# SrikarK-code/clip-dplm

Hardware: NVIDIA B200
Metric: contrastive_fwd_bwd_pairs_per_sec (higher is better)
Workload: dtype bf16

## Files before the change

### clip-dplm_b200/csrc/clipnce_api.cu

```cuda
#include <cuda.h>
#include <cuda_bf16.h>
#include <cuda_runtime.h>

#include <cmath>
#include <cstdarg>
#include <cstdio>
#include <cstdlib>
#include <cstring>
#include <mutex>
#include <set>
#include <string>
#include <utility>

#include "../../include/clipnce.h"
#include "kernels_aux.cuh"
#include "kernels_head.cuh"
#include "kernels_link.cuh"
#include "kernels_pair.cuh"
#include "kernels_pair2.cuh"
#include "kernels_simt.cuh"
#include "kernels_tc.cuh"

namespace {

thread_local std::string g_err;

int fail(int code, const char* fmt, ...) {
  char buf[512];
  va_list ap;
  va_start(ap, fmt);
  vsnprintf(buf, sizeof buf, fmt, ap);
  va_end(ap);
  g_err = buf;
  return code;
}

#define CUDA_TRY(expr)                                                                              \
  do {                                                                                              \
    cudaError_t e_ = (expr);                                                                        \
    if (e_ != cudaSuccess) return fail(CLIPNCE_ECUDA, "%s: %s", #expr, cudaGetErrorString(e_));     \
  } while (0)

long long env_int(const char* name, long long dflt) {
  const char* e = getenv(name);
  return e ? atoll(e) : dflt;
}

unsigned long long link_timeout_ns() {
  static const unsigned long long ns = [] {
    const long long ms = env_int("CLIPNCE_LINK_TIMEOUT_MS", 600000);
    return (unsigned long long)(ms > 0 ? ms : 600000) * 1000000ull;
  }();
  return ns;
}
inline cudaStream_t as_stream(void* s) { return reinterpret_cast<cudaStream_t>(s); }
inline int64_t ceil_div(int64_t a, int64_t b) { return (a + b - 1) / b; }
inline int64_t round_up(int64_t a, int64_t b) { return ceil_div(a, b) * b; }
inline bool aligned16(const void* p) { return (reinterpret_cast<uintptr_t>(p) & 15u) == 0; }
inline size_t elem_size(int dtype) { return dtype == CLIPNCE_BF16 ? 2 : 4; }

bool pair_eligible(int64_t d) { return d % 128 == 0 && d >= 128 && d <= 768; }

int tc_family(int dtype, int64_t d, float scale, int flags) {
  if (dtype != CLIPNCE_BF16 || (flags & CLIPNCE_FLAG_FORCE_EXACT) || d < 8 || d % 8 != 0 || d > 768 || !(scale > 0.f)) return 0;
  if (!(flags & CLIPNCE_FLAG_UNBOUNDED) && 2.f * scale <= 80.f) return 1;
  return pair_eligible(d) ? 2 : 0;
}
bool tc_eligible(int dtype, int64_t d, float scale, int flags) { return tc_family(dtype, d, scale, flags) == 1; }

typedef CUresult (*EncodeTiledFn)(CUtensorMap*, CUtensorMapDataType, cuuint32_t, void*, const cuuint64_t*,
                                  const cuuint64_t*, const cuuint32_t*, const cuuint32_t*, CUtensorMapInterleave,
                                  CUtensorMapSwizzle, CUtensorMapL2promotion, CUtensorMapFloatOOBfill);
std::mutex g_mu;
EncodeTiledFn g_encode = nullptr;
std::set<std::pair<const void*, int>> g_smem_allowed;

int get_encode(EncodeTiledFn* out) {
  std::lock_guard<std::mutex> lk(g_mu);
  if (!g_encode) {
    void* fn = nullptr;
    cudaDriverEntryPointQueryResult qres;
    CUDA_TRY(cudaGetDriverEntryPoint("cuTensorMapEncodeTiled", &fn, cudaEnableDefault, &qres));
    if (qres != cudaDriverEntryPointSuccess || fn == nullptr)
      return fail(CLIPNCE_ECUDA, "cuTensorMapEncodeTiled not available from this driver");
    g_encode = reinterpret_cast<EncodeTiledFn>(fn);
  }
  *out = g_encode;
  return 0;
}

int make_tmap(CUtensorMap* m, const void* base, int64_t inner, int64_t outer, int64_t ld, int box_rows) {
  EncodeTiledFn enc;
  int rc = get_encode(&enc);
  if (rc) return rc;
  cuuint64_t dims[2] = {(cuuint64_t)inner, (cuuint64_t)outer};
  cuuint64_t strides[1] = {(cuuint64_t)ld * 2};
  cuuint32_t box[2] = {64u, (cuuint32_t)box_rows};
  cuuint32_t estr[2] = {1u, 1u};
  CUresult r = enc(m, CU_TENSOR_MAP_DATA_TYPE_BFLOAT16, 2, const_cast<void*>(base), dims, strides, box, estr,
                   CU_TENSOR_MAP_INTERLEAVE_NONE, CU_TENSOR_MAP_SWIZZLE_128B, CU_TENSOR_MAP_L2_PROMOTION_L2_256B,
                   CU_TENSOR_MAP_FLOAT_OOB_FILL_NONE);
  if (r != CUDA_SUCCESS)
// ... 950 lines not shown
    }
    if (world >= 2 || forced_seg >= 1) break;
  }
  if (best_p == 0) return false;
  pl->P = best_p;
  pl->Q = slots - best_p;
  pl->n_seg = best_seg;
  pl->seg_steps = pl->n_steps / best_seg;
  pl->n_items = pl->n_rb * best_seg;
  pl->n_rounds = (int)ceil_div(pl->n_items, pl->P);
  pl->depth = pair2::RING_DEPTH;
  const int nkc = (int)(d / 64);
  const int total = (pair::SMEM_LIMIT - pair2::producer_smem(nkc, 0)) / pair::STAGE_BYTES;
  if (total < 4) return false;
  auto cap = [](int v) { return v > pair2::MAXS ? pair2::MAXS : v; };
  pl->stages_b = cap(total / 2);
  pl->stages_a = cap(total - total / 2);
  pl->stages_c = cap((pair::SMEM_LIMIT - pair2::consumer_smem(0)) / pair2::C_STAGE);
  const int ps = pair2::producer_smem(nkc, pl->stages_a + pl->stages_b), cs = pair2::consumer_smem(pl->stages_c);
  pl->smem = ps > cs ? ps : cs;
  size_t off = 0;
  auto region = [&](size_t bytes) { const size_t o = off; off = (size_t)round_up((int64_t)(off + bytes), 256); return o; };
  pl->off_flags = region(sizeof(uint32_t) * 2 * (size_t)pl->n_rounds * (size_t)pl->seg_steps);
  pl->off_ring = region((size_t)pl->depth * (size_t)pl->P * 128 * 256 * 2);
  pl->off_dxh = region(sizeof(float) * (size_t)pl->n_seg * (size_t)n_rows * (size_t)d);
  pl->off_dyh = region(sizeof(float) * (size_t)n_cols * (size_t)d);
  pl->off_part = region(sizeof(float) * (size_t)ceil_div(n_rows > n_cols ? n_rows : n_cols, 8));
  pl->bytes = off;
  return true;
}

int launch_finish(const float* parts, int n_split, int64_t slab_elems, const void* xc, const void* xo, int in_dtype,
                  const float* rinv, const float* grad_scale, int64_t n, int64_t d, void* dx, int out_dtype, float* ds_part,
                  cudaStream_t st) {
  const unsigned grid = (unsigned)ceil_div(n, 8);
  const size_t smem = sizeof(float) * 8 * (size_t)d;
  const int di = (int)d;
#define FINISH3(TI, TO)                                                                                                \
  aux::finish_rows_v4<__nv_bfloat16, TI, TO><<<grid, 256, smem, st>>>(parts, n_split, slab_elems, (const __nv_bfloat16*)xc, \
                                                                      (const TI*)xo, rinv, grad_scale, n, di, (TO*)dx, ds_part)
  if (in_dtype == CLIPNCE_BF16 && out_dtype == CLIPNCE_BF16) FINISH3(__nv_bfloat16, __nv_bfloat16);
  else if (in_dtype == CLIPNCE_BF16) FINISH3(__nv_bfloat16, float);
  else if (out_dtype == CLIPNCE_BF16) FINISH3(float, __nv_bfloat16);
  else FINISH3(float, float);
#undef FINISH3
  CUDA_TRY(cudaGetLastError());
  return 0;
}

int bwd2_launch(const Bwd2Plan& pl, const void* x, const void* y, const float* rinv_x, const float* rinv_y, int64_t n_rows,
                int64_t n_cols, int64_t d, int64_t diag_offset, float scale, const float* scale_dev, const float* row_m,
                const float* row_w, const float* col_m, const float* col_w, float diag_w, char* ws, float* const* dy_peer,
                int world, cudaStream_t st) {
  uint32_t* flags_dev = reinterpret_cast<uint32_t*>(ws + pl.off_flags);
  const size_t n_flags = (size_t)pl.n_rounds * (size_t)pl.seg_steps;
  CUDA_TRY(cudaMemsetAsync(flags_dev, 0, sizeof(uint32_t) * 2 * n_flags, st));
  pair2::Params p;
  memset(&p, 0, sizeof p);
  p.n_rows = (int)n_rows; p.n_cols = (int)n_cols; p.d = (int)d;
  p.nkc = (int)(d / 64); p.nq2 = (int)ceil_div(d, 256); p.n_half = pl.n_half;
  p.nsbuf = p.nq2 <= 2 ? 2 : 1;
  p.n_rb = pl.n_rb; p.n_seg = pl.n_seg; p.seg_steps = pl.seg_steps; p.n_items = pl.n_items; p.n_rounds = pl.n_rounds;
  p.P = pl.P; p.Q = pl.Q; p.depth = pl.depth;
  p.stages_a = pl.stages_a; p.stages_b = pl.stages_b; p.stages_c = pl.stages_c;
  p.diag_offset = diag_offset; p.scale = scale; p.scale_dev = scale_dev; p.diag_w = diag_w;
  p.rinv_x = rinv_x; p.rinv_y = rinv_y; p.row_m = row_m; p.row_w = row_w; p.col_m = col_m; p.col_w = col_w;
  p.dx = reinterpret_cast<float*>(ws + pl.off_dxh);
  p.dy = reinterpret_cast<float*>(ws + pl.off_dyh);
  p.world = world;
  for (int s = 0; s < world; ++s) p.dy_peer[s] = dy_peer[s];
  p.ready = flags_dev; p.done = flags_dev + n_flags;
  CUtensorMap tx, ty, tyg, tg;
  int rc;
  if ((rc = make_tmap(&tx, x, d, n_rows, d, pair2::ROWS))) return rc;
  if ((rc = make_tmap(&ty, y, d, n_cols, d, 128))) return rc;
  if ((rc = make_tmap(&tyg, y, d, n_cols, d, 64))) return rc;
  if ((rc = make_tmap(&tg, ws + pl.off_ring, 256, (int64_t)pl.depth * pl.P * 128, 256, 64))) return rc;
  auto kern = tc_family(CLIPNCE_BF16, d, scale, 0) == 2 ? pair2::bwd2_kernel<true> : pair2::bwd2_kernel<false>;
  if ((rc = allow_smem(kern, pair::SMEM_LIMIT))) return rc;
  kern<<<2 * (pl.P + pl.Q), pair2::THREADS, pl.smem, st>>>(tx, ty, tyg, tg, p);
  CUDA_TRY(cudaGetLastError());
  return 0;
}
}

extern "C" {

int clipnce_backward_both_workspace_bytes(int64_t n_rows, int64_t n_cols, int64_t d, int dtype, float scale, int flags,
                                          int world, size_t* out) {
  if (!out) return fail(CLIPNCE_EINVAL, "backward_both_workspace_bytes: null pointer");
  Bwd2Plan pl;
  *out = (n_rows >= 1 && n_cols >= 1 && d >= 1 && bwd2_plan(n_rows, n_cols, d, dtype, scale, flags, world, &pl) &&
          check_device_sm100() == 0 && bwd2_device_ok()) ? pl.bytes : 0;
  return 0;
}

int clipnce_backward_both_dx(const void* x, const void* y, const float* rinv_x, const float* rinv_y, int64_t n,
                             int64_t d, float scale, const float* scale_dev, const float* row_m, const float* row_w,
                             const float* col_m, const float* col_w, float diag_w, int dtype, int flags,
                             const void* x_orig, const void* y_orig, int in_dtype, const float* grad_scale, void* dx,
                             void* dy, int out_dtype, float* d_scale_sum, void* workspace, size_t workspace_bytes,
                             void* stream) {
  if (!x || !y || !rinv_x || !rinv_y || !row_m || !row_w || !col_m || !col_w || !x_orig || !y_orig || !dx || !dy || !workspace)
    return fail(CLIPNCE_EINVAL, "backward_both_dx: null pointer");
  if ((in_dtype != CLIPNCE_BF16 && in_dtype != CLIPNCE_F32) || (out_dtype != CLIPNCE_BF16 && out_dtype != CLIPNCE_F32))
    return fail(CLIPNCE_EINVAL, "backward_both_dx: bad dtype");
  if (in_dtype == dtype && (x_orig != x || y_orig != y))
    return fail(CLIPNCE_EINVAL, "backward_both_dx: x_orig / y_orig of the compute type must be x / y themselves");
  if (!aligned16(x) || !aligned16(y) || !aligned16(workspace)) return fail(CLIPNCE_EINVAL, "backward_both_dx: operands must be 16-byte aligned");
  int rc = check_device_sm100();
  if (rc) return rc;
  Bwd2Plan pl;
  if (!bwd2_plan(n, n, d, dtype, scale, flags, 0, &pl) || !bwd2_device_ok())
    return fail(CLIPNCE_EUNSUPPORTED, "backward_both_dx: shape not served (see clipnce_backward_both_workspace_bytes)");
  if (workspace_bytes < pl.bytes) return fail(CLIPNCE_EWORKSPACE, "backward_both_dx: workspace %zu < %zu", workspace_bytes, pl.bytes);
  cudaStream_t st = as_stream(stream);
  char* ws = reinterpret_cast<char*>(workspace);
  if ((rc = bwd2_launch(pl, x, y, rinv_x, rinv_y, n, n, d, 0, scale, scale_dev, row_m, row_w, col_m, col_w, diag_w, ws, nullptr,
                        0, st)))
    return rc;
  float* ds_part = reinterpret_cast<float*>(ws + pl.off_part);
  if ((rc = launch_finish(reinterpret_cast<float*>(ws + pl.off_dxh), pl.n_seg, n * d, x, x_orig, in_dtype, rinv_x, grad_scale, n, d,
                          dx, out_dtype, d_scale_sum ? ds_part : nullptr, st)))
    return rc;
  if ((rc = launch_finish(reinterpret_cast<float*>(ws + pl.off_dyh), 1, n * d, y, y_orig, in_dtype, rinv_y, grad_scale, n, d, dy,
                          out_dtype, nullptr, st)))
    return rc;
  if (d_scale_sum) {
    aux::reduce_scalar_partials_par<<<1, 256, 0, st>>>(ds_part, (int)ceil_div(n, 8), 1.f, d_scale_sum);
    CUDA_TRY(cudaGetLastError());
  }
  return 0;
}

int clipnce_backward_both_sharded(const void* x, const void* y, const float* rinv_x, const float* rinv_y, int64_t n_rows,
                                  int64_t n_cols, int64_t d, int64_t diag_offset, float scale, const float* scale_dev,
                                  const float* row_m, const float* row_w, const float* col_m, const float* col_w,
                                  float diag_w, int dtype, int flags, const void* x_orig, int in_dtype,
                                  const float* grad_scale, void* dx, int out_dtype, float* d_scale_sum,
                                  void* const* peer_base, int world, int rank, int64_t slots_offset, void* workspace,
                                  size_t workspace_bytes, void* stream) {
  if (!x || !y || !rinv_x || !rinv_y || !row_m || !row_w || !col_m || !col_w || !x_orig || !workspace || !peer_base)
    return fail(CLIPNCE_EINVAL, "backward_both_sharded: null pointer");
  if ((in_dtype != CLIPNCE_BF16 && in_dtype != CLIPNCE_F32) || (out_dtype != CLIPNCE_BF16 && out_dtype != CLIPNCE_F32))
    return fail(CLIPNCE_EINVAL, "backward_both_sharded: bad dtype");
  if (in_dtype == dtype && x_orig != x) return fail(CLIPNCE_EINVAL, "backward_both_sharded: x_orig of the compute type must be x itself");
  if (!aligned16(x) || !aligned16(y) || !aligned16(workspace)) return fail(CLIPNCE_EINVAL, "backward_both_sharded: operands must be 16-byte aligned");
  if (world < 2 || world > pair2::MAX_WORLD || rank < 0 || rank >= world || slots_offset < 0 || slots_offset % 16 != 0)
    return fail(CLIPNCE_EINVAL, "backward_both_sharded: bad world / rank / slots_offset");
  if (diag_offset != (int64_t)rank * n_rows) return fail(CLIPNCE_EINVAL, "backward_both_sharded: diag_offset must be rank * n_rows");
  int rc = check_device_sm100();
  if (rc) return rc;
  Bwd2Plan pl;
  if (!bwd2_plan(n_rows, n_cols, d, dtype, scale, flags, world, &pl) || !bwd2_device_ok())
    return fail(CLIPNCE_EUNSUPPORTED, "backward_both_sharded: shape not served (see clipnce_backward_both_workspace_bytes)");
  if (workspace_bytes < pl.bytes) return fail(CLIPNCE_EWORKSPACE, "backward_both_sharded: workspace %zu < %zu", workspace_bytes, pl.bytes);
  cudaStream_t st = as_stream(stream);
  char* ws = reinterpret_cast<char*>(workspace);
  float* dy_peer[pair2::MAX_WORLD];
  for (int s = 0; s < world; ++s) {
    if (!peer_base[s] || !aligned16(peer_base[s])) return fail(CLIPNCE_EINVAL, "backward_both_sharded: peer buffer %d is null or unaligned", s);
    dy_peer[s] = reinterpret_cast<float*>(reinterpret_cast<char*>(peer_base[s]) + slots_offset) + (size_t)rank * (size_t)n_rows * (size_t)d;
  }
  if ((rc = bwd2_launch(pl, x, y, rinv_x, rinv_y, n_rows, n_cols, d, diag_offset, scale, scale_dev, row_m, row_w, col_m, col_w,
                        diag_w, ws, dy_peer, world, st)))
    return rc;
  if (!dx) return 0;
  float* ds_part = reinterpret_cast<float*>(ws + pl.off_part);
  if ((rc = launch_finish(reinterpret_cast<float*>(ws + pl.off_dxh), pl.n_seg, n_rows * d, x, x_orig, in_dtype, rinv_x, grad_scale,
                          n_rows, d, dx, out_dtype, d_scale_sum ? ds_part : nullptr, st)))
    return rc;
  if (d_scale_sum) {
    aux::reduce_scalar_partials_par<<<1, 256, 0, st>>>(ds_part, (int)ceil_div(n_rows, 8), 1.f, d_scale_sum);
    CUDA_TRY(cudaGetLastError());
  }
  return 0;
}

int clipnce_finish_sharded(const void* x, const void* x_orig, const float* rinv_x, void* dx, const void* y_local,
                           const void* y_orig, const float* rinv_y_local, void* dy, const float* slots, int64_t n_rows,
                           int64_t n_cols, int64_t d, int dtype, float scale, int flags, int world, int in_dtype,
                           int out_dtype, const float* grad_scale, float* d_scale_sum, void* workspace,
                           size_t workspace_bytes, void* stream) {
  if (!x || !x_orig || !rinv_x || !dx || !y_local || !y_orig || !rinv_y_local || !dy || !slots || !workspace)
    return fail(CLIPNCE_EINVAL, "finish_sharded: null pointer");
  if ((in_dtype != CLIPNCE_BF16 && in_dtype != CLIPNCE_F32) || (out_dtype != CLIPNCE_BF16 && out_dtype != CLIPNCE_F32))
    return fail(CLIPNCE_EINVAL, "finish_sharded: bad dtype");
  Bwd2Plan pl;
  if (!bwd2_plan(n_rows, n_cols, d, dtype, scale, flags, world, &pl))
    return fail(CLIPNCE_EUNSUPPORTED, "finish_sharded: shape not served by the two-sided backward");
  if (workspace_bytes < pl.bytes) return fail(CLIPNCE_EWORKSPACE, "finish_sharded: workspace %zu < %zu", workspace_bytes, pl.bytes);
  cudaStream_t st = as_stream(stream);
  char* ws = reinterpret_cast<char*>(workspace);
  float* ds_part = reinterpret_cast<float*>(ws + pl.off_part);
  aux::FinishSide s0, s1;
  s0.parts = reinterpret_cast<float*>(ws + pl.off_dxh); s0.n_split = pl.n_seg; s0.slab = n_rows * d; s0.xc = x; s0.xo = x_orig;
  s0.rinv = rinv_x; s0.dx = dx; s0.ds_part = d_scale_sum ? ds_part : nullptr;
  s1.parts = slots; s1.n_split = world; s1.slab = n_rows * d; s1.xc = y_local; s1.xo = y_orig; s1.rinv = rinv_y_local; s1.dx = dy;
  s1.ds_part = nullptr;
  const dim3 grid((unsigned)ceil_div(n_rows, 8), 2);
  const size_t smem = sizeof(float) * 8 * (size_t)d;
  const int di = (int)d;
#define FINISHD(TI, TO) aux::finish_rows_v4_dual<__nv_bfloat16, TI, TO><<<grid, 256, smem, st>>>(s0, s1, grad_scale, n_rows, di)
  if (in_dtype == CLIPNCE_BF16 && out_dtype == CLIPNCE_BF16) FINISHD(__nv_bfloat16, __nv_bfloat16);
  else if (in_dtype == CLIPNCE_BF16) FINISHD(__nv_bfloat16, float);
  else if (out_dtype == CLIPNCE_BF16) FINISHD(float, __nv_bfloat16);
  else FINISHD(float, float);
#undef FINISHD
// ... 324 lines not shown
```

Before: 4.331 million.

## Add three-role persistent bwd3 kernel for single-device symmetric backward

Adds a new persistent clustered backward kernel for the symmetric n==n case. It splits CTA pairs into three roles: logits/softmax-gradient producers that write G tiles to a global ring, dx accumulators, and dy consumers that pick up ring slots through ready/done flags. A cost model chooses how many pairs go to the logits role. The aim is to overlap the dx and dy GEMMs across SMs and avoid bwd2's segmented dx partials. In exchange it adds global ring traffic, flag spinning, and read-modify-write accumulation of dy across rounds. It only runs for n>=16384, n%256==0 and d in {128..512}; otherwise it falls back to bwd2.

```diff
diff --git a/clip-dplm_b200/csrc/clipnce_api.cu b/clip-dplm_b200/csrc/clipnce_api.cu
--- a/clip-dplm_b200/csrc/clipnce_api.cu
+++ b/clip-dplm_b200/csrc/clipnce_api.cu
@@ -18,6 +18,7 @@
 #include "kernels_link.cuh"
 #include "kernels_pair.cuh"
 #include "kernels_pair2.cuh"
+#include "kernels_pair3.cuh"
 #include "kernels_simt.cuh"
 #include "kernels_tc.cuh"
 
@@ -1134,6 +1135,136 @@
   CUDA_TRY(cudaGetLastError());
   return 0;
 }
+
+struct Bwd3Plan {
+  int L, Q, n_rb, n_steps, n_rounds, n_half, depth, stages_l, stages_x, stages_c, smem;
+  size_t off_flags, off_ring, off_dxh, off_dyh, off_part, bytes;
+};
+
+bool bwd3_device_ok() {
+  if (env_int("CLIPNCE_NO_BWD3", 0) != 0) return false;
+  if (allow_smem(pair3::bwd3_kernel<false>, pair::SMEM_LIMIT) || allow_smem(pair3::bwd3_kernel<true>, pair::SMEM_LIMIT)) {
+    cudaGetLastError();
+    return false;
+  }
+  static const bool ok = [] {
+    cudaLaunchConfig_t cfg;
+    memset(&cfg, 0, sizeof cfg);
+    cfg.gridDim = dim3(2 * pair_slots());
+    cfg.blockDim = dim3(pair3::THREADS);
+    cfg.dynamicSmemBytes = pair::SMEM_LIMIT;
+    int n = 0, n2 = 0;
+    if (cudaOccupancyMaxActiveClusters(&n, pair3::bwd3_kernel<false>, &cfg) != cudaSuccess ||
+        cudaOccupancyMaxActiveClusters(&n2, pair3::bwd3_kernel<true>, &cfg) != cudaSuccess) {
+      cudaGetLastError();
+      return false;
+    }
+    return n >= pair_slots() && n2 >= pair_slots();
+  }();
+  return ok;
+}
+
+bool bwd3_plan(int64_t n, int64_t d, int dtype, float scale, int flags, Bwd3Plan* pl) {
+  const int fam = tc_family(dtype, d, scale, flags);
+  if (!(fam == 1 || fam == 2) || (flags & CLIPNCE_FLAG_UNBOUNDED) || d % 128 != 0 || d < 128 || d > 512) return false;
+  const int forced_l = (int)env_int("CLIPNCE_BWD3_L", 0);
+  constexpr int64_t kMinRows = 16384;
+  if (n % 256 != 0 || n > (1ll << 22) || (forced_l < 1 && n < kMinRows)) return false;
+  const int slots = pair_slots();
+  if (slots < 8) return false;
+  pl->n_rb = (int)(n / 256);
+  pl->n_steps = (int)(n / 256);
+  pl->n_half = (int)ceil_div(d, 256);
+  int best_l = 0;
+  if (forced_l >= 1) {
+    if (2 * forced_l > slots - 1) return false;
+    best_l = forced_l;
+  } else {
+    double best_t = 1e300;
+    for (int L = 1; 2 * L <= slots - 1 && L <= pl->n_rb; ++L) {
+      const double tl = (double)ceil_div(pl->n_rb, L) * (double)(pl->n_steps + 1);
+      const double tq = (double)pl->n_rb * (double)pl->n_steps / (double)(slots - 2 * L);
+      const double t = tl > tq ? tl : tq;
+      if (t < best_t - 1e-9) { best_t = t; best_l = L; }
+    }
+  }
+  if (best_l == 0) return false;
+  pl->L = best_l;
+  pl->Q = slots - 2 * best_l;
+  pl->n_rounds = (int)ceil_div(pl->n_rb, pl->L);
+  pl->depth = pair3::RING_DEPTH;
+  const int nkc = (int)(d / 64);
+  auto cap = [](int v) { return v > pair3::MAXS ? pair3::MAXS : v; };
+  pl->stages_l = cap((pair::SMEM_LIMIT - pair3::logits_smem(nkc, 0)) / pair::STAGE_BYTES);
+  pl->stages_x = cap((pair::SMEM_LIMIT - pair3::dx_smem((int)d, 0)) / pair3::dx_stage((int)d));
+  pl->stages_c = cap((pair::SMEM_LIMIT - pair3::dy_smem(0)) / pair3::C_STAGE);
+  if (pl->stages_l < 2 || pl->stages_x < 2 || pl->stages_c < 2) return false;
+  const int ls = pair3::logits_smem(nkc, pl->stages_l), xs = pair3::dx_smem((int)d, pl->stages_x),
+            cs = pair3::dy_smem(pl->stages_c);
+  pl->smem = ls > xs ? (ls > cs ? ls : cs) : (xs > cs ? xs : cs);
+  size_t off = 0;
+  auto region = [&](size_t bytes) { const size_t o = off; off = (size_t)round_up((int64_t)(off + bytes), 256); return o; };
+  pl->off_flags = region(sizeof(uint32_t) * 2 * (size_t)pl->n_rounds * (size_t)pl->n_steps);
+  pl->off_ring = region((size_t)pl->depth * (size_t)pl->L * 256 * 256 * 2);
+  pl->off_dxh = region(sizeof(float) * (size_t)n * (size_t)d);
+  pl->off_dyh = region(sizeof(float) * (size_t)n * (size_t)d);
+  pl->off_part = region(sizeof(float) * (size_t)ceil_div(n, 8));
+  pl->bytes = off;
+  return true;
+}
+
+int bwd3_launch(const Bwd3Plan& pl, const void* x, const void* y, const float* rinv_x, const float* rinv_y, int64_t n, int64_t d,
+                float scale, const float* scale_dev, const float* row_m, const float* row_w, const float* col_m,
+                const float* col_w, float diag_w, char* ws, cudaStream_t st) {
+  uint32_t* flags_dev = reinterpret_cast<uint32_t*>(ws + pl.off_flags);
+  const size_t n_flags = (size_t)pl.n_rounds * (size_t)pl.n_steps;
+  CUDA_TRY(cudaMemsetAsync(flags_dev, 0, sizeof(uint32_t) * 2 * n_flags, st));
+  pair3::Params p;
+  memset(&p, 0, sizeof p);
+  p.n = (int)n; p.d = (int)d;
+  p.nkc = (int)(d / 64); p.nq2 = (int)ceil_div(d, 256); p.n_half = pl.n_half;
+  p.n_rb = pl.n_rb; p.n_steps = pl.n_steps; p.n_rounds = pl.n_rounds;
+  p.L = pl.L; p.Q = pl.Q; p.depth = pl.depth;
+  p.stages_l = pl.stages_l; p.stages_x = pl.stages_x; p.stages_c = pl.stages_c;
+  p.small_off = pl.smem - pair3::SMALL;
+  p.scale = scale; p.scale_dev = scale_dev; p.diag_w = diag_w;
+  p.rinv_x = rinv_x; p.rinv_y = rinv_y; p.row_m = row_m; p.row_w = row_w; p.col_m = col_m; p.col_w = col_w;
+  p.dx = reinterpret_cast<float*>(ws + pl.off_dxh);
+  p.dy = reinterpret_cast<float*>(ws + pl.off_dyh);
+  p.ring = reinterpret_cast<uint8_t*>(ws + pl.off_ring);
+  p.ready = flags_dev; p.done = flags_dev + n_flags;
+  CUtensorMap tx, txg, ty, tyg, tg, tgt;
+  const int64_t ring_rows = (int64_t)pl.depth * pl.L * 256;
+  int rc;
+  if ((rc = make_tmap(&tx, x, d, n, d, 128))) return rc;
+  if ((rc = make_tmap(&txg, x, d, n, d, 64))) return rc;
+  if ((rc = make_tmap(&ty, y, d, n, d, 128))) return rc;
+  if ((rc = make_tmap(&tyg, y, d, n, d, 64))) return rc;
+  if ((rc = make_tmap(&tg, ws + pl.off_ring, 256, ring_rows, 256, 128))) return rc;
+  if ((rc = make_tmap(&tgt, ws + pl.off_ring, 256, ring_rows, 256, 64))) return rc;
+  auto kern = tc_family(CLIPNCE_BF16, d, scale, 0) == 2 ? pair3::bwd3_kernel<true> : pair3::bwd3_kernel<false>;
+  if ((rc = allow_smem(kern, pair::SMEM_LIMIT))) return rc;
+  kern<<<2 * (2 * pl.L + pl.Q), pair3::THREADS, pl.smem, st>>>(tx, txg, ty, tyg, tg, tgt, p);
+  CUDA_TRY(cudaGetLastError());
+  return 0;
+}
+
+struct BothRoute {
+  bool three;
+  Bwd3Plan p3;
+  Bwd2Plan p2;
+  size_t bytes;
+};
+bool both_route(int64_t n, int64_t d, int dtype, float scale, int flags, BothRoute* rt) {
+  rt->three = bwd3_plan(n, d, dtype, scale, flags, &rt->p3) && check_device_sm100() == 0 && bwd3_device_ok();
+  if (rt->three) {
+    rt->bytes = rt->p3.bytes;
+    return true;
+  }
+  if (!bwd2_plan(n, n, d, dtype, scale, flags, 0, &rt->p2) || check_device_sm100() != 0 || !bwd2_device_ok()) return false;
+  rt->bytes = rt->p2.bytes;
+  return true;
+}
 }
 
 extern "C" {
@@ -1141,9 +1272,16 @@
 int clipnce_backward_both_workspace_bytes(int64_t n_rows, int64_t n_cols, int64_t d, int dtype, float scale, int flags,
                                           int world, size_t* out) {
   if (!out) return fail(CLIPNCE_EINVAL, "backward_both_workspace_bytes: null pointer");
+  *out = 0;
+  if (n_rows < 1 || n_cols < 1 || d < 1) return 0;
+  if (world == 0) {
+    BothRoute rt;
+    if (n_rows == n_cols && both_route(n_rows, d, dtype, scale, flags, &rt)) *out = rt.bytes;
+    return 0;
+  }
   Bwd2Plan pl;
-  *out = (n_rows >= 1 && n_cols >= 1 && d >= 1 && bwd2_plan(n_rows, n_cols, d, dtype, scale, flags, world, &pl) &&
-          check_device_sm100() == 0 && bwd2_device_ok()) ? pl.bytes : 0;
+  *out = (bwd2_plan(n_rows, n_cols, d, dtype, scale, flags, world, &pl) && check_device_sm100() == 0 && bwd2_device_ok())
+             ? pl.bytes : 0;
   return 0;
 }
 
@@ -1162,20 +1300,27 @@
   if (!aligned16(x) || !aligned16(y) || !aligned16(workspace)) return fail(CLIPNCE_EINVAL, "backward_both_dx: operands must be 16-byte aligned");
   int rc = check_device_sm100();
   if (rc) return rc;
-  Bwd2Plan pl;
-  if (!bwd2_plan(n, n, d, dtype, scale, flags, 0, &pl) || !bwd2_device_ok())
+  BothRoute rt;
+  if (!both_route(n, d, dtype, scale, flags, &rt))
     return fail(CLIPNCE_EUNSUPPORTED, "backward_both_dx: shape not served (see clipnce_backward_both_workspace_bytes)");
-  if (workspace_bytes < pl.bytes) return fail(CLIPNCE_EWORKSPACE, "backward_both_dx: workspace %zu < %zu", workspace_bytes, pl.bytes);
+  if (workspace_bytes < rt.bytes) return fail(CLIPNCE_EWORKSPACE, "backward_both_dx: workspace %zu < %zu", workspace_bytes, rt.bytes);
   cudaStream_t st = as_stream(stream);
   char* ws = reinterpret_cast<char*>(workspace);
-  if ((rc = bwd2_launch(pl, x, y, rinv_x, rinv_y, n, n, d, 0, scale, scale_dev, row_m, row_w, col_m, col_w, diag_w, ws, nullptr,
-                        0, st)))
-    return rc;
-  float* ds_part = reinterpret_cast<float*>(ws + pl.off_part);
-  if ((rc = launch_finish(reinterpret_cast<float*>(ws + pl.off_dxh), pl.n_seg, n * d, x, x_orig, in_dtype, rinv_x, grad_scale, n, d,
+  if (rt.three) {
+    rc = bwd3_launch(rt.p3, x, y, rinv_x, rinv_y, n, d, scale, scale_dev, row_m, row_w, col_m, col_w, diag_w, ws, st);
+  } else {
+    rc = bwd2_launch(rt.p2, x, y, rinv_x, rinv_y, n, n, d, 0, scale, scale_dev, row_m, row_w, col_m, col_w, diag_w, ws, nullptr, 0,
+                     st);
+  }
+  if (rc) return rc;
+  const int n_seg = rt.three ? 1 : rt.p2.n_seg;
+  const size_t off_dxh = rt.three ? rt.p3.off_dxh : rt.p2.off_dxh, off_dyh = rt.three ? rt.p3.off_dyh : rt.p2.off_dyh,
+               off_part = rt.three ? rt.p3.off_part : rt.p2.off_part;
+  float* ds_part = reinterpret_cast<float*>(ws + off_part);
+  if ((rc = launch_finish(reinterpret_cast<float*>(ws + off_dxh), n_seg, n * d, x, x_orig, in_dtype, rinv_x, grad_scale, n, d,
                           dx, out_dtype, d_scale_sum ? ds_part : nullptr, st)))
     return rc;
-  if ((rc = launch_finish(reinterpret_cast<float*>(ws + pl.off_dyh), 1, n * d, y, y_orig, in_dtype, rinv_y, grad_scale, n, d, dy,
+  if ((rc = launch_finish(reinterpret_cast<float*>(ws + off_dyh), 1, n * d, y, y_orig, in_dtype, rinv_y, grad_scale, n, d, dy,
                           out_dtype, nullptr, st)))
     return rc;
   if (d_scale_sum) {
diff --git a/clip-dplm_b200/csrc/kernels_pair3.cuh b/clip-dplm_b200/csrc/kernels_pair3.cuh
--- /dev/null
+++ b/clip-dplm_b200/csrc/kernels_pair3.cuh
@@ -0,0 +1,587 @@
+#pragma once
+#include "kernels_pair2.cuh"
+
+namespace pair3 {
+
+using pair::LOG2E;
+using pair::STAGE_BYTES;
+using pair::STEP_J;
+using pair::TMEM_COLS;
+
+constexpr int THREADS = 640;
+constexpr int EPI_WARPS = 16;
+constexpr int DY_EPI_WARPS = 8;
+constexpr int FLAG_WARP = 3;
+constexpr int ROWS = 128;
+constexpr int X_CHUNK = ROWS * 128;
+constexpr int G_BOX = 16384;
+constexpr int SMALL = 10240;
+constexpr int C_STAGE = 32768;
+constexpr int FLUSH_BYTES = DY_EPI_WARPS * 4096;
+constexpr int MAXS = 6;
+constexpr int RING_DEPTH = 16;
+
+constexpr int B_FULL = 0, B_EMPTY = MAXS, B_XFULL = 2 * MAXS, B_XEMPTY = B_XFULL + 1, B_SFULL = B_XEMPTY + 1,
+              B_SEMPTY = B_SFULL + 2, B_GWRITTEN = B_SEMPTY + 2, B_SLOTFREE = B_GWRITTEN + 1, B_ACCFULL = B_SLOTFREE + 1,
+              B_ACCEMPTY = B_ACCFULL + 2, B_STEPFULL = B_ACCEMPTY + 2, B_STEPEMPTY = B_STEPFULL + 2,
+              B_COUNT = B_STEPEMPTY + 2;
+static_assert(B_COUNT * 8 <= 1000, "barrier block");
+
+struct Params {
+  int n, d;
+  int nkc, nq2, n_half;
+  int n_rb, n_steps, n_rounds;
+  int L, Q, depth;
+  int stages_l, stages_x, stages_c;
+  int small_off;
+  float scale, diag_w;
+  const float* scale_dev;
+  const float* rinv_x;
+  const float* rinv_y;
+  const float* row_m;
+  const float* row_w;
+  const float* col_m;
+  const float* col_w;
+  float* dx;
+  float* dy;
+  uint8_t* ring;
+  uint32_t* ready;
+  uint32_t* done;
+};
+
+__host__ __device__ constexpr int logits_smem(int nkc, int stages) {
+  return nkc * X_CHUNK + stages * STAGE_BYTES + SMALL;
+}
+__host__ __device__ constexpr int dx_stage(int d) { return G_BOX + 64 * d; }
+__host__ __device__ constexpr int dx_smem(int d, int stages) { return stages * dx_stage(d) + SMALL; }
+__host__ __device__ constexpr int dy_smem(int stages) { return stages * C_STAGE + FLUSH_BYTES + SMALL; }
+
+__device__ __forceinline__ void st_global_v8_hint(void* p, uint32_t a0, uint32_t a1, uint32_t a2, uint32_t a3, uint32_t a4,
+                                                  uint32_t a5, uint32_t a6, uint32_t a7, uint64_t policy) {
+  asm volatile("st.global.L2::cache_hint.v8.b32 [%0], {%1, %2, %3, %4, %5, %6, %7, %8}, %9;"
+               ::"l"(p), "r"(a0), "r"(a1), "r"(a2), "r"(a3), "r"(a4), "r"(a5), "r"(a6), "r"(a7), "l"(policy)
+               : "memory");
+}
+
+__device__ __forceinline__ int round_items(const Params& p, int r) { return min(p.L, p.n_rb - r * p.L); }
+__device__ __forceinline__ uint32_t readers(const Params& p, int r) { return (uint32_t)(p.n_half + round_items(p, r)); }
+
+template <bool TWO_EXP>
+__global__ void __cluster_dims__(2, 1, 1) __launch_bounds__(THREADS, 1)
+bwd3_kernel(const __grid_constant__ CUtensorMap tmap_x,
+            const __grid_constant__ CUtensorMap tmap_xg,
+            const __grid_constant__ CUtensorMap tmap_y,
+            const __grid_constant__ CUtensorMap tmap_yg,
+            const __grid_constant__ CUtensorMap tmap_g,
+            const __grid_constant__ CUtensorMap tmap_gt,
+            const Params p) {
+  extern __shared__ __align__(1024) uint8_t smem[];
+  const uint32_t base = ptx::smem_u32(smem);
+  if ((base & 1023u) != 0) __trap();
+  const uint32_t rank = ptx::cluster_ctarank();
+  const bool leader = rank == 0;
+  const int warp = threadIdx.x >> 5;
+  const int lane = threadIdx.x & 31;
+  const int pair_id = blockIdx.x >> 1;
+  const int role = pair_id < p.L ? 0 : (pair_id < 2 * p.L ? 1 : 2);
+
+  const uint32_t bars = base + p.small_off;
+  auto bar = [&](int i) -> uint32_t { return bars + 8u * i; };
+  volatile uint32_t* tmem_ptr_smem = reinterpret_cast<volatile uint32_t*>(smem + p.small_off + 1016);
+  float* const colv = reinterpret_cast<float*>(smem + p.small_off + 1024);
+
+  const float sc = p.scale_dev != nullptr ? __ldg(p.scale_dev) : p.scale;
+  const float k2 = sc * LOG2E;
+
+  if (warp == 0 && lane == 0) {
+    ptx::prefetch_tmap(&tmap_x);
+    ptx::prefetch_tmap(&tmap_xg);
+    ptx::prefetch_tmap(&tmap_y);
+    ptx::prefetch_tmap(&tmap_yg);
+    ptx::prefetch_tmap(&tmap_g);
+    ptx::prefetch_tmap(&tmap_gt);
+  }
+  if (warp == 1 && lane == 0) {
+    for (int s = 0; s < MAXS; ++s) {
+      ptx::mbar_init(bar(B_FULL + s), 1);
+      ptx::mbar_init(bar(B_EMPTY + s), 1);
+    }
+    ptx::mbar_init(bar(B_XFULL), 1);
+    ptx::mbar_init(bar(B_XEMPTY), 1);
+    for (int b = 0; b < 2; ++b) {
+      ptx::mbar_init(bar(B_SFULL + b), 1);
+      ptx::mbar_init(bar(B_SEMPTY + b), 2 * EPI_WARPS);
+      ptx::mbar_init(bar(B_ACCFULL + b), 1);
+      ptx::mbar_init(bar(B_ACCEMPTY + b), 2 * (role == 1 ? EPI_WARPS : DY_EPI_WARPS));
+      ptx::mbar_init(bar(B_STEPFULL + b), 1);
+      ptx::mbar_init(bar(B_STEPEMPTY + b), 1);
+    }
+    ptx::mbar_init(bar(B_GWRITTEN), EPI_WARPS);
+    ptx::mbar_init(bar(B_SLOTFREE), 1);
+    ptx::fence_mbar_init();
+  }
+  if (warp == 2) ptx::tmem_alloc_pair(ptx::smem_u32(const_cast<uint32_t*>(tmem_ptr_smem)), TMEM_COLS);
+  ptx::tc_fence_before();
+  __syncthreads();
+  ptx::cluster_sync();
+  ptx::tc_fence_after();
+  const uint32_t tmem_base = *tmem_ptr_smem;
+
+  const uint32_t desc_hi_k = static_cast<uint32_t>(ptx::smem_desc_k_sw128(0) >> 32);
+  const uint32_t desc_hi_mn = static_cast<uint32_t>(ptx::smem_desc_mn_sw128(0, 8192) >> 32);
+  auto desc_lo = [&](uint32_t addr, uint32_t lbo16) -> uint32_t { return ((addr & 0x3FFFFu) >> 4) | (lbo16 << 16); };
+  auto mk = [&](uint32_t hi, uint32_t lo) -> uint64_t { return (static_cast<uint64_t>(hi) << 32) | lo; };
+
+  if (role == 0) {
+    const uint32_t x_smem = base;
+    const uint32_t ring_a = x_smem + p.nkc * X_CHUNK;
+
+    if (warp == 0) {
+      if (ptx::elect_one()) {
+        int stage = 0;
+        uint32_t phase = 0;
+        for (int r = 0; r < p.n_rounds; ++r) {
+          const int item = r * p.L + pair_id;
+          if (item >= p.n_rb) break;
+          const int i0 = item * STEP_J + (int)rank * ROWS;
+          ptx::mbar_wait(bar(B_XEMPTY), (r & 1) ^ 1u);
+          if (leader) ptx::mbar_arrive_expect_tx(bar(B_XFULL), 2 * p.nkc * X_CHUNK);
+          for (int kc = 0; kc < p.nkc; ++kc)
+            ptx::tma_load_2d_pair(x_smem + kc * X_CHUNK, &tmap_x, bar(B_XFULL), kc * 64, i0);
+          for (int t = 0; t < p.n_steps; ++t) {
+            for (int g = 0; g < p.nkc; ++g) {
+              ptx::mbar_wait(bar(B_EMPTY + stage), phase ^ 1u);
+              if (leader) ptx::mbar_arrive_expect_tx(bar(B_FULL + stage), 2 * STAGE_BYTES);
+              ptx::tma_load_2d_pair(ring_a + stage * STAGE_BYTES, &tmap_y, bar(B_FULL + stage), g * 64,
+                                    t * STEP_J + (int)rank * 128);
+              if (++stage == p.stages_l) { stage = 0; phase ^= 1u; }
+            }
+          }
+        }
+      }
+      __syncwarp();
+    } else if (warp == 1) {
+      if (leader && ptx::elect_one()) {
+        constexpr uint32_t idesc_s = ptx::idesc_bf16_f32_major(2 * ROWS, STEP_J, 0, 0);
+        const uint32_t x_lo0 = desc_lo(x_smem, 1), a_lo0 = desc_lo(ring_a, 1);
+        int stage = 0;
+        uint32_t phase = 0, ready = 0, gs = 0;
+        for (int r = 0; r < p.n_rounds; ++r) {
+          if (r * p.L + pair_id >= p.n_rb) break;
+          ptx::mbar_wait(bar(B_XFULL), r & 1);
+          for (int t = 0; t < p.n_steps; ++t, ++gs) {
+            const int sb = gs & 1;
+            ptx::mbar_wait(bar(B_SEMPTY + sb), ((gs >> 1) & 1) ^ 1u);
+            const uint32_t d_tmem = tmem_base + sb * STEP_J;
+            for (int g = 0; g < p.nkc; ++g) {
+              if (!ready) ptx::mbar_wait(bar(B_FULL + stage), phase);
+              ptx::tc_fence_after();
+              int ns = stage + 1;
+              uint32_t np = phase;
+              if (ns == p.stages_l) { ns = 0; np ^= 1u; }
+              ready = ptx::mma_box_pair(d_tmem, mk(desc_hi_k, x_lo0 + g * (X_CHUNK >> 4)),
+                                        mk(desc_hi_k, a_lo0 + stage * (STAGE_BYTES >> 4)), 2, 2, idesc_s, g != 0,
+                                        bar(B_FULL + ns), np);
+              ptx::mma_commit_pair(bar(B_EMPTY + stage));
+              if (g == p.nkc - 1) ptx::mma_commit_pair(bar(B_SFULL + sb));
+              stage = ns;
+              phase = np;
+            }
+          }
+          ptx::mma_commit_pair(bar(B_XEMPTY));
+        }
+      }
+      __syncwarp();
+    } else if (warp == FLAG_WARP) {
+      if (ptx::elect_one()) {
+        uint32_t gs = 0;
+        for (int r = 0; r < p.n_rounds; ++r) {
+          if (r * p.L + pair_id >= p.n_rb) break;
+          for (int t = 0; t < p.n_steps; ++t, ++gs) {
+            const uint32_t g = (uint32_t)r * (uint32_t)p.n_steps + (uint32_t)t;
+            if (g >= (uint32_t)p.depth) {
+              const uint32_t go = g - (uint32_t)p.depth;
+              ptx::spin_until_ge(p.done + go, readers(p, (int)(go / (uint32_t)p.n_steps)));
+            }
+            ptx::mbar_arrive(bar(B_SLOTFREE));
+            ptx::mbar_wait(bar(B_GWRITTEN), gs & 1u);
+            __threadfence();
+            pair2::publish(p.ready + g);
+          }
+        }
+      }
+      __syncwarp();
+    } else if (warp >= 4) {
+      const int e = warp - 4;
+      const int q = warp & 3;
+      const int cw = e >> 2;
+      const int i_local = 32 * q + lane;
+      const int te = threadIdx.x - 128;
+      const uint32_t t_lane = tmem_base + (static_cast<uint32_t>(q * 32) << 16);
+      const uint32_t sempty_leader = ptx::mapa(bar(B_SEMPTY), 0);
+      const uint64_t keep = ptx::l2_policy_evict_last();
+      uint32_t gs = 0;
+
+      for (int r = 0; r < p.n_rounds; ++r) {
+        const int item = r * p.L + pair_id;
+        if (item >= p.n_rb) break;
+        const int i_glob = item * STEP_J + (int)rank * ROWS + i_local;
+        const float rx = p.rinv_x[i_glob];
+        const float u = TWO_EXP ? 0.f : p.row_w[i_glob] * pair::ex2((sc - p.row_m[i_glob]) * LOG2E);
+        const float rm2 = TWO_EXP ? p.row_m[i_glob] * LOG2E : 0.f;
+        const float rw = TWO_EXP ? p.row_w[i_glob] : 0.f;
+        float cw_n = 0.f, cm_n = 0.f, ry_n = 0.f;
+        if (te < STEP_J) { cw_n = p.col_w[te]; cm_n = p.col_m[te]; ry_n = p.rinv_y[te]; }
+
+        auto form = [&](const uint32_t (&rr)[32], const float* cv, int t, int jl0, uint32_t (&pk)[16]) {
+          const int dl = i_glob - (t * STEP_J + jl0);
+          const bool has_diag = dl >= 0 && dl < 32;
+          const float* const cjp = cv + jl0;
+#pragma unroll
+          for (int x4 = 0; x4 < 8; ++x4) {
+            const float4 cj4 = *reinterpret_cast<const float4*>(cjp + 4 * x4);
+            const float4 vr4 = *reinterpret_cast<const float4*>(cjp + 256 + 4 * x4);
+            const float4 ry4 = *reinterpret_cast<const float4*>(cjp + 512 + 4 * x4);
+            const float cjv[4] = {cj4.x, cj4.y, cj4.z, cj4.w};
+            const float vrv[4] = {vr4.x, vr4.y, vr4.z, vr4.w};
+            const float ryv[4] = {ry4.x, ry4.y, ry4.z, ry4.w};
+            float g[4];
+            if constexpr (TWO_EXP) {
+              const float4 cm4 = *reinterpret_cast<const float4*>(cjp + 768 + 4 * x4);
+              const float cmv[4] = {cm4.x, cm4.y, cm4.z, cm4.w};
+#pragma unroll
+              for (int xx = 0; xx < 4; ++xx) {
+                const float y = __uint_as_float(rr[4 * x4 + xx]) * rx;
+                const float er = pair::ex2(fmaf(y, cjv[xx], -rm2)) * rw;
+                const float ec = pair::ex2(fmaf(y, cjv[xx], -cmv[xx]));
+                g[xx] = rx * fmaf(er, ryv[xx], ec * vrv[xx]);
+              }
+            } else {
+#pragma unroll
+              for (int xx = 0; xx < 4; ++xx) {
+                const float y = __uint_as_float(rr[4 * x4 + xx]) * rx;
+                const float ev = pair::ex2(fmaf(y, cjv[xx], -k2)) * rx;
+                g[xx] = ev * fmaf(u, ryv[xx], vrv[xx]);
+              }
+            }
+            if (has_diag) {
+#pragma unroll
+              for (int xx = 0; xx < 4; ++xx)
+                if (dl == 4 * x4 + xx) g[xx] -= p.diag_w * rx * ryv[xx];
+            }
+            const __nv_bfloat162 p0 = __floats2bfloat162_rn(g[0], g[1]);
+            const __nv_bfloat162 p1 = __floats2bfloat162_rn(g[2], g[3]);
+            pk[2 * x4] = *reinterpret_cast<const uint32_t*>(&p0);
+            pk[2 * x4 + 1] = *reinterpret_cast<const uint32_t*>(&p1);
+          }
+        };
+        auto put = [&](const uint32_t (&pk)[16], uint8_t* dst) {
+          st_global_v8_hint(dst, pk[0], pk[1], pk[2], pk[3], pk[4], pk[5], pk[6], pk[7], keep);
+          st_global_v8_hint(dst + 32, pk[8], pk[9], pk[10], pk[11], pk[12], pk[13], pk[14], pk[15], keep);
+        };
+
+        for (int t = 0; t < p.n_steps; ++t, ++gs) {
+          const int sb = gs & 1;
+          float* const cv = colv + (gs & 1) * 1024;
+          if (te < STEP_J) {
+            cv[te] = ry_n * k2;
+            cv[256 + te] = (TWO_EXP ? cw_n : cw_n * pair::ex2((sc - cm_n) * LOG2E)) * ry_n;
+            cv[512 + te] = ry_n;
+            if (TWO_EXP) cv[768 + te] = cw_n > 0.f ? cm_n * LOG2E : 0.f;
+            if (t + 1 < p.n_steps) {
+              const int jn = (t + 1) * STEP_J + te;
+              cw_n = p.col_w[jn]; cm_n = p.col_m[jn]; ry_n = p.rinv_y[jn];
+            }
+          }
+          pair::named_bar_sync(1, EPI_WARPS * 32);
+
+          ptx::mbar_wait(bar(B_SFULL + sb), (gs >> 1) & 1);
+          ptx::tc_fence_after();
+          uint32_t pk[16];
+          {
+            uint32_t rr[32];
+            ptx::tmem_ld_32x32b_x32(t_lane + sb * STEP_J + 32 * cw, rr);
+            ptx::tmem_ld_wait();
+            form(rr, cv, t, 32 * cw, pk);
+          }
+          uint32_t rr[32];
+          ptx::tmem_ld_32x32b_x32(t_lane + sb * STEP_J + 128 + 32 * cw, rr);
+          ptx::tmem_ld_wait();
+          ptx::tc_fence_before();
+          __syncwarp();
+          if (lane == 0) ptx::mbar_arrive_cluster(sempty_leader + 8u * sb);
+          const uint32_t g = (uint32_t)r * (uint32_t)p.n_steps + (uint32_t)t;
+          uint8_t* const row = p.ring + ((size_t)((int)(g % (uint32_t)p.depth) * p.L + pair_id) * STEP_J + (size_t)rank * ROWS +
+                                         (size_t)i_local) * (STEP_J * 2) + 2 * 32 * cw;
+          ptx::mbar_wait(bar(B_SLOTFREE), gs & 1u);
+          put(pk, row);
+          form(rr, cv, t, 128 + 32 * cw, pk);
+          put(pk, row + 2 * 128);
+          __syncwarp();
+          if (lane == 0) ptx::mbar_arrive(bar(B_GWRITTEN));
+        }
+      }
+    }
+  } else if (role == 1) {
+    const int partner = pair_id - p.L;
+    const int xs = dx_stage(p.d);
+
+    if (warp == 0) {
+      if (ptx::elect_one()) {
+        int stage = 0;
+        uint32_t phase = 0;
+        const uint64_t keep = ptx::l2_policy_evict_last();
+        for (int r = 0; r < p.n_rounds; ++r) {
+          if (r * p.L + partner >= p.n_rb) break;
+          const uint32_t pw2 = 2u * (uint32_t)round_items(p, r);
+          for (int t = 0; t < p.n_steps; ++t) {
+            const uint32_t g = (uint32_t)r * (uint32_t)p.n_steps + (uint32_t)t;
+            const int grow = ((int)(g % (uint32_t)p.depth) * p.L + partner) * STEP_J + (int)rank * ROWS;
+            ptx::spin_until_ge(p.ready + g, pw2);
+            ptx::fence_proxy_async_all();
+            for (int kc = 0; kc < 4; ++kc) {
+              ptx::mbar_wait(bar(B_EMPTY + stage), phase ^ 1u);
+              if (leader) ptx::mbar_arrive_expect_tx(bar(B_FULL + stage), 2 * xs);
+              const uint32_t st = base + stage * xs;
+              ptx::tma_load_2d_pair_hint(st, &tmap_g, bar(B_FULL + stage), 64 * kc, grow, keep);
+              for (int q2 = 0; q2 < p.nq2; ++q2) {
+                const int half = min(256, p.d - 256 * q2) >> 1;
+                for (int gi = 0; gi < (half >> 6); ++gi)
+                  ptx::tma_load_2d_pair(st + G_BOX + 16384 * q2 + 8192 * gi, &tmap_yg, bar(B_FULL + stage),
+                                        256 * q2 + half * (int)rank + 64 * gi, t * STEP_J + 64 * kc);
+              }
+              if (++stage == p.stages_x) { stage = 0; phase ^= 1u; }
+            }
+          }
+        }
+      }
+      __syncwarp();
+    } else if (warp == 1) {
+      if (leader && ptx::elect_one()) {
+        const uint32_t a_lo0 = desc_lo(base, 1), b_lo0 = desc_lo(base + G_BOX, 8192 >> 4);
+        int stage = 0;
+        uint32_t phase = 0, ready = 0, sg = 0, it = 0;
+        for (int r = 0; r < p.n_rounds; ++r, ++it) {
+          if (r * p.L + partner >= p.n_rb) break;
+          ptx::mbar_wait(bar(B_ACCEMPTY), (it & 1) ^ 1u);
+          ptx::tc_fence_after();
+          for (int t = 0; t < p.n_steps; ++t, ++sg) {
+            for (int kc = 0; kc < 4; ++kc) {
+              if (!ready) ptx::mbar_wait(bar(B_FULL + stage), phase);
+              ptx::tc_fence_after();
+              int ns = stage + 1;
+              uint32_t np = phase;
+              if (ns == p.stages_x) { ns = 0; np ^= 1u; }
+              const uint32_t so = (uint32_t)(stage * xs) >> 4;
+              for (int q2 = 0; q2 < p.nq2; ++q2) {
+                const int wq = min(256, p.d - 256 * q2);
+                const uint32_t idesc = ptx::idesc_bf16_f32_major(2 * ROWS, wq, 0, 1);
+                const bool last = q2 == p.nq2 - 1;
+                const uint32_t rdy = ptx::mma_box_pair(tmem_base + 256 * q2, mk(desc_hi_k, a_lo0 + so),
+                                                       mk(desc_hi_mn, b_lo0 + so + 1024 * q2), 2, 2048 >> 4, idesc,
+                                                       (t | kc) != 0, bar(B_FULL + (last ? ns : stage)), last ? np : phase);
+                if (last) ready = rdy;
+              }
+              ptx::mma_commit_pair(bar(B_EMPTY + stage));
+              stage = ns;
+              phase = np;
+            }
+            ptx::mbar_wait(bar(B_STEPEMPTY + (sg & 1)), ((sg >> 1) & 1) ^ 1u);
+            ptx::mma_commit_pair(bar(B_STEPFULL + (sg & 1)));
+          }
+          ptx::mma_commit_pair(bar(B_ACCFULL));
+        }
+      }
+      __syncwarp();
+    } else if (warp == FLAG_WARP) {
+      if (leader && ptx::elect_one()) {
+        uint32_t sg = 0;
+        for (int r = 0; r < p.n_rounds; ++r) {
+          if (r * p.L + partner >= p.n_rb) break;
+          for (int t = 0; t < p.n_steps; ++t, ++sg) {
+            ptx::mbar_wait(bar(B_STEPFULL + (sg & 1)), (sg >> 1) & 1);
+            ptx::tc_fence_after();
+            ptx::red_release_gpu_add(p.done + ((uint32_t)r * (uint32_t)p.n_steps + (uint32_t)t), 1u);
+            ptx::mbar_arrive(bar(B_STEPEMPTY + (sg & 1)));
+          }
+        }
+      }
+      __syncwarp();
+    } else if (warp >= 4) {
+      const int q = warp & 3;
+      const int cg = (warp - 4) >> 2;
+      const uint32_t t_lane = tmem_base + (static_cast<uint32_t>(q * 32) << 16);
+      const uint32_t accempty_leader = ptx::mapa(bar(B_ACCEMPTY), 0);
+      uint32_t it = 0;
+      for (int r = 0; r < p.n_rounds; ++r, ++it) {
+        const int item = r * p.L + partner;
+        if (item >= p.n_rb) break;
+        const int i_glob = item * STEP_J + (int)rank * ROWS + 32 * q + lane;
+        const float osc = sc / p.rinv_x[i_glob];
+        ptx::mbar_wait(bar(B_ACCFULL), it & 1);
+        ptx::tc_fence_after();
+        float* const dst = p.dx + (long long)i_glob * p.d;
+        for (int c32 = cg; c32 < (p.d >> 5); c32 += 4) {
+          uint32_t rr[32];
+          ptx::tmem_ld_32x32b_x32(t_lane + 32 * c32, rr);
+          ptx::tmem_ld_wait();
+#pragma unroll
+          for (int x4 = 0; x4 < 8; ++x4)
+            *reinterpret_cast<float4*>(dst + 32 * c32 + 4 * x4) =
+                make_float4(__uint_as_float(rr[4 * x4]) * osc, __uint_as_float(rr[4 * x4 + 1]) * osc,
+                            __uint_as_float(rr[4 * x4 + 2]) * osc, __uint_as_float(rr[4 * x4 + 3]) * osc);
+        }
+        ptx::tc_fence_before();
+        __syncwarp();
+        if (lane == 0) ptx::mbar_arrive_cluster(accempty_leader);
+      }
+    }
+  } else {
+    const int cidx = pair_id - 2 * p.L;
+    const uint32_t ring_c = base;
+
+    if (warp == 0) {
+      if (ptx::elect_one()) {
+        int stage = 0;
+        uint32_t phase = 0;
+        const uint64_t keep = ptx::l2_policy_evict_last();
+        for (int r = 0; r < p.n_rounds; ++r) {
+          const int pw = round_items(p, r);
+          for (int t = 0; t < p.n_steps; ++t) {
+            const uint32_t g = (uint32_t)r * (uint32_t)p.n_steps + (uint32_t)t;
+            const int slot = (int)(g % (uint32_t)p.depth);
+            bool step_ready = false;
+            for (int hh = 0; hh < p.n_half; ++hh) {
+              if ((t * p.n_half + hh) % p.Q != cidx) continue;
+              if (!step_ready) {
+                ptx::spin_until_ge(p.ready + g, 2u * (uint32_t)pw);
+                ptx::fence_proxy_async_all();
+                step_ready = true;
+              }
+              const int wq = min(256, p.d - 256 * hh);
+              const int ngr = wq >> 7;
+              for (int pp = 0; pp < pw; ++pp) {
+                for (int kb = 0; kb < 4; ++kb) {
+                  ptx::mbar_wait(bar(B_EMPTY + stage), phase ^ 1u);
+                  if (leader) ptx::mbar_arrive_expect_tx(bar(B_FULL + stage), 2 * (2 + ngr) * 8192);
+                  const uint32_t st = ring_c + stage * C_STAGE;
+                  const int grow = (slot * p.L + pp) * STEP_J + 64 * kb;
+                  const int xrow = (r * p.L + pp) * STEP_J + 64 * kb;
+                  for (int gi = 0; gi < 2; ++gi)
+                    ptx::tma_load_2d_pair_hint(st + gi * 8192, &tmap_gt, bar(B_FULL + stage), 128 * (int)rank + 64 * gi, grow, keep);
+                  for (int gi = 0; gi < ngr; ++gi)
+                    ptx::tma_load_2d_pair(st + 16384 + gi * 8192, &tmap_xg, bar(B_FULL + stage),
+                                          256 * hh + (wq >> 1) * (int)rank + 64 * gi, xrow);
+                  if (++stage == p.stages_c) { stage = 0; phase ^= 1u; }
+                }
+              }
+            }
+          }
+        }
+      }
+      __syncwarp();
+    } else if (warp == 1) {
+      if (leader && ptx::elect_one()) {
+        const uint32_t a_lo0 = desc_lo(ring_c, 8192 >> 4), b_lo0 = desc_lo(ring_c + 16384, 8192 >> 4);
+        int stage = 0;
+        uint32_t phase = 0, ready = 0, nt = 0;
+        for (int r = 0; r < p.n_rounds; ++r) {
+          const int nk = 4 * round_items(p, r);
+          for (int t = 0; t < p.n_steps; ++t) {
+            for (int hh = 0; hh < p.n_half; ++hh) {
+              if ((t * p.n_half + hh) % p.Q != cidx) continue;
+              const int buf = nt & 1;
+              ptx::mbar_wait(bar(B_ACCEMPTY + buf), ((nt >> 1) & 1) ^ 1u);
+              ptx::tc_fence_after();
+              const int wq = min(256, p.d - 256 * hh);
+              const uint32_t idesc = ptx::idesc_bf16_f32_major(256, wq, 1, 1);
+              const uint32_t d_tmem = tmem_base + buf * 256;
+              for (int kk = 0; kk < nk; ++kk) {
+                if (!ready) ptx::mbar_wait(bar(B_FULL + stage), phase);
+                ptx::tc_fence_after();
+                int ns = stage + 1;
+                uint32_t np = phase;
+                if (ns == p.stages_c) { ns = 0; np ^= 1u; }
+                ready = ptx::mma_box_pair(d_tmem, mk(desc_hi_mn, a_lo0 + stage * (C_STAGE >> 4)),
+                                          mk(desc_hi_mn, b_lo0 + stage * (C_STAGE >> 4)), 2048 >> 4, 2048 >> 4, idesc,
+                                          kk != 0, bar(B_FULL + ns), np);
+                ptx::mma_commit_pair(bar(B_EMPTY + stage));
+                stage = ns;
+                phase = np;
+              }
+              ptx::mma_commit_pair(bar(B_ACCFULL + buf));
+              ++nt;
+            }
+          }
+        }
+      }
+      __syncwarp();
+    } else if (warp >= 4 && warp < 4 + DY_EPI_WARPS) {
+      const int q = warp & 3;
+      const int hcol = (warp - 4) >> 2;
+      const uint32_t t_lane = tmem_base + (static_cast<uint32_t>(q * 32) << 16);
+      const uint32_t accempty_leader = ptx::mapa(bar(B_ACCEMPTY), 0);
+      const uint32_t scratch = ring_c + p.stages_c * C_STAGE + (warp - 4) * 4096;
+      uint32_t nt = 0;
+      for (int r = 0; r < p.n_rounds; ++r) {
+        for (int t = 0; t < p.n_steps; ++t) {
+          for (int hh = 0; hh < p.n_half; ++hh) {
+            if ((t * p.n_half + hh) % p.Q != cidx) continue;
+            const int buf = nt & 1;
+            const long long j = (long long)t * STEP_J + (int)rank * 128 + 32 * q + lane;
+            const float osc = sc / p.rinv_y[j];
+            ptx::mbar_wait(bar(B_ACCFULL + buf), (nt >> 1) & 1);
+            ptx::tc_fence_after();
+            if (leader && warp == 4 && lane == 0)
+              ptx::red_release_gpu_add(p.done + ((uint32_t)r * (uint32_t)p.n_steps + (uint32_t)t), 1u);
+            const int wq = min(256, p.d - 256 * hh);
+            const int wh = wq >> 1;
+            const long long col0 = 256 * hh + hcol * wh;
+            const long long j0 = j - lane;
+            float* const obase = p.dy + j0 * p.d + col0;
+            const int rsub = lane >> 3, ch = lane & 7;
+            for (int c = 0; c < (wh >> 5); ++c) {
+              uint32_t rr[32];
+              ptx::tmem_ld_32x32b_x32(t_lane + buf * 256 + hcol * wh + 32 * c, rr);
+              ptx::tmem_ld_wait();
+#pragma unroll
+              for (int k4 = 0; k4 < 8; ++k4)
+                pair::st_shared_v4(scratch + lane * 128 + ((static_cast<uint32_t>(k4) ^ (lane & 7)) << 4),
+                                   __float_as_uint(__uint_as_float(rr[4 * k4]) * osc), __float_as_uint(__uint_as_float(rr[4 * k4 + 1]) * osc),
+                                   __float_as_uint(__uint_as_float(rr[4 * k4 + 2]) * osc), __float_as_uint(__uint_as_float(rr[4 * k4 + 3]) * osc));
+              __syncwarp();
+              float4 v[8];
+#pragma unroll
+              for (int i = 0; i < 8; ++i) {
+                const int row = 4 * i + rsub;
+                v[i] = pair2::ld_shared_v4(scratch + row * 128 + ((static_cast<uint32_t>(ch) ^ (row & 7)) << 4));
+              }
+              if (r > 0) {
+#pragma unroll
+                for (int i = 0; i < 8; ++i) {
+                  const float4 old = *reinterpret_cast<const float4*>(obase + (long long)(4 * i + rsub) * p.d + 32 * c + 4 * ch);
+                  v[i].x += old.x; v[i].y += old.y; v[i].z += old.z; v[i].w += old.w;
+                }
+              }
+#pragma unroll
+              for (int i = 0; i < 8; ++i)
+                *reinterpret_cast<float4*>(obase + (long long)(4 * i + rsub) * p.d + 32 * c + 4 * ch) = v[i];
+              __syncwarp();
+            }
+            ptx::tc_fence_before();
+            __syncwarp();
+            if (lane == 0) ptx::mbar_arrive_cluster(accempty_leader + 8u * buf);
+            ++nt;
+          }
+        }
+      }
+    }
+  }
+
+  ptx::tc_fence_before();
+  __syncthreads();
+  ptx::cluster_sync();
+  if (warp == 2) ptx::tmem_dealloc_pair(tmem_base, TMEM_COLS);
+}
+
+}
```

New measurement: 3.586 million, median of 6. 17.2% lower.
